# evroon/mav-detection

Hardware: NVIDIA B200
Metric: 1080p frame-pairs/sec (flow+FoE+mask) (higher is better)
Workload: dtype f32

## Files before the change

mav_detection_b200/csrc/api.cu:

```cuda
#include <math.h>
#include <stdarg.h>
#include <stdlib.h>
#include <string.h>

#include <algorithm>
#include <new>
#include <vector>

#include "common.cuh"

namespace mavd {

static thread_local char g_err[512] = "";
std::atomic<int64_t> g_launches{0};

void set_error(const char* fmt, ...) {
    va_list ap;
    va_start(ap, fmt);
    vsnprintf(g_err, sizeof(g_err), fmt, ap);
    va_end(ap);
}

static inline int cv_round(double v) { return (int)nearbyint(v); }

// ... 568 lines not shown
    pdl_break(h, 0);
    pdl_break(h, 1);
    MAVD_REQUIRE(n >= 0 && n <= h->cfg.max_pairs, MAVD_ERR_INVALID, "%s: batch %d exceeds max_pairs %d", what, n,
                 h->cfg.max_pairs);
    return MAVD_OK;
}

static void note_farneback_call(mavd_handle h, const uint8_t* d_frames, int n_pairs, int pair_stride, float* d_flow) {
    h->last_pairs = n_pairs;
    h->last_stride = pair_stride;
    h->last_flow0 = d_flow;
    h->last_frames = d_frames;
}

int mavd_farneback_tap(mavd_handle h, int32_t kind, int32_t level, int32_t index, float* d_out, void* stream) {
    MAVD_REQUIRE(h && d_out, MAVD_ERR_INVALID, "tap: NULL argument");
    DeviceGuard dg(h->cfg.device);
    MAVD_REQUIRE(index >= 0 && index < h->max_frames, MAVD_ERR_INVALID, "tap: index out of range");
    return farneback_tap(h, kind, level, index, d_out, (cudaStream_t)stream);
}

static int upload_imu(mavd_handle h, const mavd_imu* h_imu, int n, cudaStream_t s, int* n64, int* n32) {
    MAVD_REQUIRE(h_imu != nullptr, MAVD_ERR_INVALID, "imu array is NULL");
    int a = 0, b = 0, rot = 0;
    for (int i = 0; i < n; ++i) {
        if (h_imu[i].derotate) {
            MAVD_REQUIRE(h_imu[i].dt != 0.0, MAVD_ERR_INVALID, "imu[%d].dt is zero", i);
            ++a;
            if (!(h_imu[i].ang[0] == 0.0 && h_imu[i].ang[1] == 0.0 && h_imu[i].ang[2] == 0.0)) ++rot;
        } else {
            ++b;
        }
    }
    if (n64) *n64 = a;
    if (n32) *n32 = b;
    h->batch_rot = rot;
    const int k = h->imu_next;
    h->imu_next = (k + 1) % mavd_handle_s::kImuRing;
    MAVD_CUDA(cudaEventSynchronize(h->imu_ev[k]));
    mavd_imu* stage = h->h_imu_ring + (size_t)k * h->cfg.max_pairs;
    memcpy(stage, h_imu, sizeof(mavd_imu) * n);
    MAVD_CUDA(cudaMemcpyAsync(h->d_imu, stage, sizeof(mavd_imu) * n, cudaMemcpyHostToDevice, s));
    MAVD_CUDA(cudaEventRecord(h->imu_ev[k], s));
    return MAVD_OK;
}

int mavd_derotate(mavd_handle h, const float* d_flow, int32_t n, const mavd_imu* h_imu, double* d_out, void* stream) {
    DeviceGuard dg(h ? h->cfg.device : -1);
    TRY(check_batch(h, n, "derotate"));
    if (n == 0) return MAVD_OK;
    MAVD_REQUIRE(d_flow && d_out, MAVD_ERR_INVALID, "derotate: NULL buffer");
    TRY(upload_imu(h, h_imu, n, (cudaStream_t)stream, nullptr, nullptr));
    return derotate_run(h, d_flow, 0, n, h->d_imu, d_out, (cudaStream_t)stream);
}

int mavd_derotate_f64(mavd_handle h, const double* d_flow, int32_t n, const mavd_imu* h_imu, double* d_out, void* stream) {
    DeviceGuard dg(h ? h->cfg.device : -1);
    TRY(check_batch(h, n, "derotate_f64"));
    if (n == 0) return MAVD_OK;
// ... 51 lines not shown

int mavd_debug_force_exact_residual(mavd_handle h, int32_t on) {
    MAVD_REQUIRE(h != nullptr, MAVD_ERR_INVALID, "handle is NULL");
    DeviceGuard dg(h->cfg.device);
    MAVD_CUDA(cudaDeviceSynchronize());
    drop_graphs(h);
    h->force_exact_residual = on != 0;
    return MAVD_OK;
}

int mavd_residual_masks(mavd_handle h, const float* d_flow, int32_t n, const mavd_imu* h_imu,
                        const mavd_detect_params* prm, const double* d_foe, const uint8_t* d_sky, int64_t sky_stride,
                        const uint8_t* d_seg, int64_t seg_stride, void* d_phi, uint8_t* d_total, uint8_t* d_fixed,
                        mavd_frame_stats* d_stats, void* stream) {
    DeviceGuard dg(h ? h->cfg.device : -1);
    TRY(check_batch(h, n, "residual_masks"));
    if (n == 0) return MAVD_OK;
    MAVD_REQUIRE(d_flow && d_foe, MAVD_ERR_INVALID, "residual_masks: NULL buffer");
    mavd_detect_params p;
    if (prm) p = *prm; else mavd_default_detect_params(&p);
    int n64 = 0, n32 = 0;
    TRY(upload_imu(h, h_imu, n, (cudaStream_t)stream, &n64, &n32));
    return residual_run(h, d_flow, 0, n, h->d_imu, p, d_foe, d_sky, sky_stride, d_seg, seg_stride, d_phi, d_total, d_fixed,
                        d_stats, sizeof(mavd_frame_stats), n64 > 0 ? (h->batch_rot > 0 ? 1 : 2) : 0, n32 > 0, (cudaStream_t)stream);
}

static int check_det(mavd_handle h, int max_det, const void* det, const char* what) {
    if (!det) return MAVD_OK;
    MAVD_REQUIRE(max_det >= 1 && max_det <= MAVD_MAX_DETECTIONS, MAVD_ERR_INVALID, "%s: max_det %d outside 1..%d", what,
                 max_det, MAVD_MAX_DETECTIONS);
    MAVD_REQUIRE((reinterpret_cast<uintptr_t>(det) & 7) == 0, MAVD_ERR_INVALID, "%s: detections must be 8-byte aligned",
                 what);
    if (h->d_det_area) return MAVD_OK;
    mavd_handle_full* H = static_cast<mavd_handle_full*>(h);
    TRY(H->arena.alloc(&H->d_det_area, (size_t)h->cfg.max_pairs * det_lab_stride(h)));
    TRY(H->arena.alloc(&H->d_det_nlabels, (size_t)h->cfg.max_pairs));
    H->bytes = H->arena.bytes;
    return MAVD_OK;
}

int mavd_detections(mavd_handle h, const uint8_t* d_mask, int32_t n, const float* d_flow, const mavd_imu* h_imu,
                    int32_t max_det, mavd_detection* d_det, void* stream) {
    DeviceGuard dg(h ? h->cfg.device : -1);
    TRY(check_batch(h, n, "detections"));
    MAVD_REQUIRE(d_det != nullptr, MAVD_ERR_INVALID, "detections: NULL table");
    MAVD_REQUIRE(!d_flow || h_imu, MAVD_ERR_INVALID, "detections: a flow needs an imu array");
    TRY(check_det(h, max_det, d_det, "detections"));
// ... 69 lines not shown
static int detect_run(mavd_handle h, const float* flow, int n, const mavd_detect_params& p, int n64, int n32,
                      const int32_t* d_samples, const mavd_aux_inputs& aux, uint8_t* d_total_out, uint8_t* fixed,
                      mavd_frame_record* d_records, int max_det, mavd_detection* d_det, cudaStream_t s) {
    char* stats0 = reinterpret_cast<char*>(d_records) + offsetof(mavd_frame_record, stats);
    const bool fork = h->s_aux != nullptr && !h->prof.on;
    if (fork) {
        MAVD_CUDA(cudaEventRecord(h->ev_fork, s));
        MAVD_CUDA(cudaStreamWaitEvent(h->s_aux, h->ev_fork, 0));
        pdl_break(h, 1);
        TRY(ccl_list_reset(h, n, h->s_aux, 1));
        TRY(residual_prepare(h, n, aux.seg, aux.seg_stride, reinterpret_cast<mavd_frame_stats*>(stats0),
                             sizeof(mavd_frame_record), h->s_aux, 1));
        MAVD_CUDA(cudaEventRecord(h->ev_join, h->s_aux));
    }
    TRY(foe_run(h, flow, 0, n, h->d_imu, p, d_samples, h->d_foe, h->d_ninter, s));
    if (fork) {
        MAVD_CUDA(cudaStreamWaitEvent(s, h->ev_join, 0));
        pdl_break(h, 0);
    } else {
        TRY(ccl_list_reset(h, n, s));
    }
    TRY(residual_run(h, flow, 0, n, h->d_imu, p, h->d_foe, aux.sky, aux.sky_stride, aux.seg, aux.seg_stride, nullptr,
                     d_total_out, fixed, reinterpret_cast<mavd_frame_stats*>(stats0), sizeof(mavd_frame_record),
                     n64 > 0 ? (h->batch_rot > 0 ? 1 : 2) : 0, n32 > 0, s, true, aux.gt_flow, fork));
    int32_t* boxes0 = reinterpret_cast<int32_t*>(reinterpret_cast<char*>(d_records) + offsetof(mavd_frame_record, boxes));
    char* nl0 = reinterpret_cast<char*>(d_records) + offsetof(mavd_frame_record, n_labels);
    const DetArgs da{d_det, max_det, h->d_det_area, det_lab_stride(h), flow, h->d_imu};
    TRY(ccl_run(h, fixed, n, nullptr, boxes0, sizeof(mavd_frame_record) / sizeof(int32_t), MAVD_MAX_BOXES,
                reinterpret_cast<int32_t*>(nl0), sizeof(mavd_frame_record), s, true, d_det ? &da : nullptr));
    MAVD_CUDA(launch_chained(pdl_next(h), records_fill_kernel, ceil_div(n, 128), 128, 0, s, d_records, h->d_foe, h->d_ninter, n));
    MAVD_LAUNCHED();
    return MAVD_OK;
}

}

static constexpr size_t kMaxGraphs = 16;

struct KeyBuilder {
    std::vector<uint64_t> k;
    KeyBuilder& operator()(const void* p) { k.push_back((uint64_t)(uintptr_t)p); return *this; }
    KeyBuilder& operator()(int64_t v) { k.push_back((uint64_t)v); return *this; }
    KeyBuilder& operator()(const mavd_detect_params& p) {
        const size_t n = sizeof(p) / sizeof(uint64_t);
        uint64_t w[sizeof(mavd_detect_params) / sizeof(uint64_t)];
        memcpy(w, &p, sizeof(p));
        k.insert(k.end(), w, w + n);
// ... 95 lines not shown
    MAVD_REQUIRE(d_frames && d_flow, MAVD_ERR_INVALID, "farneback: NULL buffer");
    StreamScope ss(h, stream);
    note_farneback_call(h, d_frames, n_pairs, pair_stride, d_flow);
    return run_graphed(h, std::move(KeyBuilder()(int64_t(1))(d_frames)(int64_t(n_pairs))(int64_t(pair_stride))(d_flow).k),
                       ss.s, [&](cudaStream_t s) { return farneback_run(h, d_frames, n_pairs, pair_stride, d_flow, s); });
}

int mavd_detect_det(mavd_handle h, const float* d_flow, int32_t n, const mavd_imu* h_imu, const mavd_detect_params* prm,
                    const int32_t* d_samples, const mavd_aux_inputs* d_aux, uint8_t* d_total_out, uint8_t* d_fixed_out,
                    mavd_frame_record* d_records, int32_t max_det, mavd_detection* d_det, void* stream) {
    DeviceGuard dg(h ? h->cfg.device : -1);
    TRY(check_batch(h, n, "detect"));
    TRY(check_det(h, max_det, d_det, "detect"));
    if (!d_det) max_det = 0;
    if (n == 0) return MAVD_OK;
    MAVD_REQUIRE(d_flow && d_samples && d_records, MAVD_ERR_INVALID, "detect: NULL buffer");
    StreamScope ss(h, stream);
    mavd_detect_params p;
    if (prm) p = *prm; else mavd_default_detect_params(&p);
    const mavd_aux_inputs aux = d_aux ? *d_aux : kNoAux;
    int n64 = 0, n32 = 0;
    TRY(upload_imu(h, h_imu, n, ss.s, &n64, &n32));
    uint8_t* fixed = d_fixed_out ? d_fixed_out : h->d_fixed;
    return run_graphed(h, std::move(KeyBuilder()(int64_t(2))(d_flow)(int64_t(n))(p)(int64_t(n64))(int64_t(h->batch_rot > 0))(int64_t(n32))(d_samples)(aux)
                                        (d_total_out)(fixed)(d_records)(int64_t(max_det))(d_det).k),
                       ss.s, [&](cudaStream_t s) {
                           return detect_run(h, d_flow, n, p, n64, n32, d_samples, aux, d_total_out, fixed, d_records,
                                             max_det, d_det, s);
                       });
}

int mavd_detect_ex(mavd_handle h, const float* d_flow, int32_t n, const mavd_imu* h_imu, const mavd_detect_params* prm,
                   const int32_t* d_samples, const mavd_aux_inputs* d_aux, uint8_t* d_total_out, uint8_t* d_fixed_out,
                   mavd_frame_record* d_records, void* stream) {
    return mavd_detect_det(h, d_flow, n, h_imu, prm, d_samples, d_aux, d_total_out, d_fixed_out, d_records, 0, nullptr,
                           stream);
}

int mavd_detect(mavd_handle h, const float* d_flow, int32_t n, const mavd_imu* h_imu, const mavd_detect_params* prm,
                const int32_t* d_samples, const uint8_t* d_sky, int64_t sky_stride, const uint8_t* d_seg,
                int64_t seg_stride, uint8_t* d_total_out, uint8_t* d_fixed_out, mavd_frame_record* d_records,
                void* stream) {
    const mavd_aux_inputs aux = {d_sky, sky_stride, d_seg, seg_stride, nullptr};
    return mavd_detect_ex(h, d_flow, n, h_imu, prm, d_samples, &aux, d_total_out, d_fixed_out, d_records, stream);
}

int mavd_process_det(mavd_handle h, const uint8_t* d_frames, int32_t n_pairs, int32_t pair_stride, const mavd_imu* h_imu,
                     const mavd_detect_params* prm, const int32_t* d_samples, const mavd_aux_inputs* d_aux,
                     float* d_flow_out, uint8_t* d_total_out, uint8_t* d_fixed_out, mavd_frame_record* d_records,
                     int32_t max_det, mavd_detection* d_det, void* stream) {
    DeviceGuard dg(h ? h->cfg.device : -1);
    TRY(check_batch(h, n_pairs, "process"));
    MAVD_REQUIRE(pair_stride == 1 || pair_stride == 2, MAVD_ERR_INVALID, "pair_stride must be 1 or 2");
    TRY(check_det(h, max_det, d_det, "process"));
    if (!d_det) max_det = 0;
    if (n_pairs == 0) return MAVD_OK;
    MAVD_REQUIRE(d_frames && d_samples && d_records, MAVD_ERR_INVALID, "process: NULL buffer");
    StreamScope ss(h, stream);
    mavd_detect_params p;
    if (prm) p = *prm; else mavd_default_detect_params(&p);
    const mavd_aux_inputs aux = d_aux ? *d_aux : kNoAux;
    float* flow = d_flow_out ? d_flow_out : h->d_flow;
    uint8_t* fixed = d_fixed_out ? d_fixed_out : h->d_fixed;
    int n64 = 0, n32 = 0;
    TRY(upload_imu(h, h_imu, n_pairs, ss.s, &n64, &n32));
    note_farneback_call(h, d_frames, n_pairs, pair_stride, flow);
    return run_graphed(h, std::move(KeyBuilder()(int64_t(3))(d_frames)(int64_t(n_pairs))(int64_t(pair_stride))(p)(int64_t(n64))(int64_t(h->batch_rot > 0))
                                        (int64_t(n32))(d_samples)(aux)(flow)(d_total_out)(fixed)(d_records)(int64_t(max_det))
                                        (d_det).k),
                       ss.s, [&](cudaStream_t s) {
                           TRY(farneback_run(h, d_frames, n_pairs, pair_stride, flow, s));
                           return detect_run(h, flow, n_pairs, p, n64, n32, d_samples, aux, d_total_out, fixed, d_records,
                                             max_det, d_det, s);
                       });
}

int mavd_process_ex(mavd_handle h, const uint8_t* d_frames, int32_t n_pairs, int32_t pair_stride, const mavd_imu* h_imu,
                    const mavd_detect_params* prm, const int32_t* d_samples, const mavd_aux_inputs* d_aux,
                    float* d_flow_out, uint8_t* d_total_out, uint8_t* d_fixed_out, mavd_frame_record* d_records,
                    void* stream) {
    return mavd_process_det(h, d_frames, n_pairs, pair_stride, h_imu, prm, d_samples, d_aux, d_flow_out, d_total_out,
                            d_fixed_out, d_records, 0, nullptr, stream);
}

int mavd_process(mavd_handle h, const uint8_t* d_frames, int32_t n_pairs, int32_t pair_stride, const mavd_imu* h_imu,
                 const mavd_detect_params* prm, const int32_t* d_samples, const uint8_t* d_sky, int64_t sky_stride,
                 const uint8_t* d_seg, int64_t seg_stride, float* d_flow_out, uint8_t* d_total_out,
                 uint8_t* d_fixed_out, mavd_frame_record* d_records, void* stream) {
    const mavd_aux_inputs aux = {d_sky, sky_stride, d_seg, seg_stride, nullptr};
    return mavd_process_ex(h, d_frames, n_pairs, pair_stride, h_imu, prm, d_samples, &aux, d_flow_out, d_total_out,
// ... 278 lines not shown
```

mav_detection_b200/csrc/common.cuh:

```cuda
#pragma once
#include <cuda.h>
#include <cuda_runtime.h>
#include <stdint.h>
#include <stdio.h>
#include <atomic>
#include <vector>

#include "mavd.h"

namespace mavd {

void set_error(const char* fmt, ...);
extern std::atomic<int64_t> g_launches;

#define MAVD_CUDA(expr)                                                                         \
    do {                                                                                        \
        cudaError_t e__ = (expr);                                                               \
        if (e__ != cudaSuccess) {                                                               \
            ::mavd::set_error("%s:%d: %s -> %s", __FILE__, __LINE__, #expr, cudaGetErrorString(e__)); \
            return (e__ == cudaErrorMemoryAllocation) ? MAVD_ERR_NOMEM : MAVD_ERR_CUDA;          \
        }                                                                                       \
    } while (0)

#define MAVD_LAUNCHED()                                                                         \
// ... 181 lines not shown
        cudaEvent_t ev_in = nullptr, ev_done = nullptr, ev_out = nullptr;
        bool busy = false;
    } slot[MAVD_HOST_SLOTS];
    cudaStream_t s_in = nullptr, s_out = nullptr;
    cudaStream_t s_aux = nullptr;
    cudaEvent_t ev_fork = nullptr, ev_join = nullptr, ev_pyr = nullptr;
    mavd_tuning tune;
    mavd::Profiler prof;
    static constexpr int kImuRing = 8;
    mavd_imu* h_imu_ring = nullptr;
    cudaEvent_t imu_ev[kImuRing] = {};
    int imu_next = 0;
    struct GraphEntry {
        std::vector<uint64_t> key;
        cudaGraphExec_t exec = nullptr;
        int64_t launches = 0;
        uint64_t last_use = 0;
    };
    std::vector<GraphEntry> graphs;
    uint64_t graph_clock = 0;
    cudaStream_t s_main = nullptr;
    cudaEvent_t ev_main_in = nullptr, ev_main_out = nullptr;
    bool force_generic_iter = false;
    int batch_rot = 0;
    bool pdl_ok[2] = {false, false};
    int last_pairs = 0, last_stride = 1;
    float* last_flow0 = nullptr;
    const uint8_t* last_frames = nullptr;
};

namespace mavd {
static inline bool pdl_next(mavd_handle h, int lane = 0) {
    const bool chained = h->tune.use_pdl != 0 && !h->prof.on && h->pdl_ok[lane];
    h->pdl_ok[lane] = true;
    return chained;
}
static inline void pdl_break(mavd_handle h, int lane = 0) { h->pdl_ok[lane] = false; }

bool encode_tensor_map_3d(CUtensorMap* map, bool is_u8, const void* base, uint64_t d0, uint64_t d1, uint64_t d2,
                          uint64_t s1_bytes, uint64_t s2_bytes, uint32_t b0, uint32_t b1, uint32_t b2);
int farneback_run(mavd_handle h, const uint8_t* d_frames, int n_pairs, int pair_stride, float* d_flow,
                  cudaStream_t s);
int farneback_tap(mavd_handle h, int kind, int level, int index, float* d_out, cudaStream_t s);
int bgr2gray_run(const uint8_t* d_bgr, uint8_t* d_gray, int64_t n, cudaStream_t s);
int derotate_run(mavd_handle h, const void* d_flow, int flow_is_f64, int n, const mavd_imu* d_imu, double* d_out,
                 cudaStream_t s);
int foe_run(mavd_handle h, const void* d_flow, int flow_kind, int n, const mavd_imu* d_imu,
// ... 40 lines not shown
```

mav_detection_b200/csrc/detect.cu:

```cuda
#include <math.h>

#include <algorithm>

#include "common.cuh"

namespace mavd {

__global__ void __launch_bounds__(256) bgr2gray_kernel(const uint8_t* __restrict__ bgr, uint8_t* __restrict__ gray,
                                                      int64_t n) {
    int64_t i4 = ((int64_t)blockIdx.x * blockDim.x + threadIdx.x) * 4;
    if (i4 >= n) return;
    if (i4 + 4 <= n && ((uintptr_t)bgr & 3) == 0 && ((uintptr_t)gray & 3) == 0) {
        const uint32_t* p = reinterpret_cast<const uint32_t*>(bgr + i4 * 3);
        uint32_t a = __ldg(p), b = __ldg(p + 1), c = __ldg(p + 2);
        uint8_t v[12];
        v[0] = a; v[1] = a >> 8; v[2] = a >> 16; v[3] = a >> 24;
        v[4] = b; v[5] = b >> 8; v[6] = b >> 16; v[7] = b >> 24;
        v[8] = c; v[9] = c >> 8; v[10] = c >> 16; v[11] = c >> 24;
        uint32_t out = 0;
#pragma unroll
        for (int k = 0; k < 4; ++k) {
            uint32_t g = (v[3 * k] * 3735u + v[3 * k + 1] * 19235u + v[3 * k + 2] * 9798u + 16384u) >> 15;
            out |= g << (8 * k);
        }
        *reinterpret_cast<uint32_t*>(gray + i4) = out;
// ... 393 lines not shown
                                           bool& m_fixed) {
    const float a2 = fmaf(fx, fx, fy * fy), b2 = fmaf(dx, dx, dy * dy);
    const float ab2 = a2 * b2;
    const bool gt_dyn = a2 > p.dyn_mm2, gt_fix = a2 > p.fix_mm2;
    bool undecided = !(a2 < 1e15f) | !(b2 < 1e15f);
    undecided |= (fabsf(a2 - p.dyn_mm2) <= p.dyn_mm2_guard) | (fabsf(a2 - p.fix_mm2) <= p.fix_mm2_guard);
    const float dot = fmaf(fx, dx, fy * dy), crs = fabsf(fmaf(fx, dy, -(fy * dx)));
    const float sf = crs * p.fix_cos - dot * p.fix_sin;
    const float thr = fmaf(p.dyn_gain, rsqrtf(a2), p.dyn_c0);
    const float tr = thr * 0.017453292519943295f;
    float sn, cs;
    __sincosf(tr, &sn, &cs);
    const float sd = crs * cs - dot * sn;
    const float mf = 3.6e-5f, md = 3.6e-5f + 1e-5f * tr;
    undecided |= (gt_dyn | gt_fix) & (ab2 < 1e-8f);
    undecided |= gt_fix & (sf * sf <= (mf * mf) * ab2);
    undecided |= gt_dyn & ((sd * sd <= (md * md) * ab2) | !(thr < 170.f));
    m_fixed = gt_fix & (sf > 0.f);
    m_total = gt_dyn & (sd > 0.f);
    return !undecided;
}

constexpr int RES_ITEMS = 4;

template <int MODE, bool FAST, int VEC, int MINB = 4>
__global__ void __launch_bounds__(256, MINB) residual_kernel(const ResidualArgs A, const FastPrm fp) {
    pdl_entry();
    const int f = blockIdx.y;
    DerotRow dr;
    dr.on = 0;
    if (MODE != 2) {
        mavd_imu im;
        im.derotate = 0;
        if (A.imu) im = A.imu[f];
        if ((im.derotate != 0) != (MODE == 0)) return;
        if (MODE == 0) {
            __shared__ double s_dr[5];
            if (threadIdx.x < 3) s_dr[threadIdx.x] = __ddiv_rn(im.ang[threadIdx.x], im.dt);
            else if (threadIdx.x == 3) s_dr[3] = __ddiv_rn(__dmul_rn((double)A.w, im.dt), 2.0);
            else if (threadIdx.x == 4) s_dr[4] = __ddiv_rn(__dmul_rn((double)A.h, im.dt), 2.0);
            __syncthreads();
            dr.o0 = s_dr[0]; dr.o1 = s_dr[1]; dr.o2 = s_dr[2]; dr.s0 = s_dr[3]; dr.s1 = s_dr[4];
            dr.on = !(dr.o0 == 0.0 && dr.o1 == 0.0 && dr.o2 == 0.0 && fabs(dr.s0) < 1e300 && fabs(dr.s1) < 1e300);
        }
    }
    const int w = A.w, h = A.h;
    const int npx = w * h;
    const int ngrp = npx / VEC;
    const double foex = A.foe[2 * f], foey = A.foe[2 * f + 1];
    const size_t fbase = (size_t)f * npx;
    const uint8_t* sky = A.sky ? A.sky + (size_t)f * A.sky_stride : nullptr;
    const uint8_t* seg = A.seg ? A.seg + (size_t)f * A.seg_stride : nullptr;
    const bool want_stats = A.stats_base != nullptr;
    int seg_min = 0;
    if (seg && want_stats) {
        const double thr = 0.1 * (double)A.seg_max[f];
        seg_min = (int)floor(thr) + 1;
    }

    int c_tot = 0, c_fix = 0, c_pos = 0, c_tpt = 0, c_fpt = 0, c_tpf = 0, c_fpf = 0, n_px = 0;
    int bx0 = 0x7fffffff, by0 = 0x7fffffff, bx1 = -1, by1 = -1;
    double sfx = 0.0, sfy = 0.0, gfx = 0.0, gfy = 0.0, maxphi = 0.0;

#pragma unroll 1
    for (int it = 0; it < RES_ITEMS; ++it) {
        const int q = (blockIdx.x * RES_ITEMS + it) * 256 + threadIdx.x;
        if (q >= ngrp) break;
        const int i0 = q * VEC;
        const int y = A.row_magic ? (int)__umulhi((unsigned)i0, A.row_magic) : i0 / w, x0 = i0 - y * w;
        double vx[VEC], vy[VEC];
        float vfx[VEC], vfy[VEC];
        if (MODE == 2) {
            const double2* fl = reinterpret_cast<const double2*>(A.flow) + fbase + i0;
#pragma unroll
            for (int k = 0; k < VEC; ++k) { const double2 v = fl[k]; vx[k] = v.x; vy[k] = v.y; }
        } else if (VEC == 4) {
            const float4* fl = reinterpret_cast<const float4*>(reinterpret_cast<const float2*>(A.flow) + fbase + i0);
            const float4 u0 = __ldg(fl), u1 = __ldg(fl + 1);
            vfx[0] = u0.x; vfy[0] = u0.y; vfx[1] = u0.z; vfy[1] = u0.w;
            vfx[2] = u1.x; vfy[2] = u1.y; vfx[3] = u1.z; vfy[3] = u1.w;
        } else {
            const float2 v = reinterpret_cast<const float2*>(A.flow)[fbase + i0];
            vfx[0] = v.x; vfy[0] = v.y;
        }
        unsigned skyw = 0, segw = 0;
        if (VEC == 4) {
            if (sky) skyw = __ldg(reinterpret_cast<const unsigned*>(sky + i0));
            if (seg) segw = __ldg(reinterpret_cast<const unsigned*>(seg + i0));
        } else {
            if (sky) skyw = sky[i0];
            if (seg) segw = seg[i0];
        }
        double yn = 0.0;
        if (MODE == 0 && dr.on) yn = __ldg(A.yn + y);
        const float dyf = (float)((double)y - foey), dxf0 = (float)((double)x0 - foex);
        unsigned totw = 0, fixw = 0;
#pragma unroll
        for (int k = 0; k < VEC; ++k) {
            const int x = x0 + k;
            const bool not_sky = ((skyw >> (8 * k)) & 255u) == 0;
            bool mt = false, mf = false;
            if (MODE == 1) {
                float phi;
                pixel_exact_f32(vfx[k], vfy[k], x, y, foex, foey, A.prm, not_sky, mt, mf, phi);
                maxphi = fmax(maxphi, (double)phi);
                if (A.phi_out) reinterpret_cast<float*>(reinterpret_cast<double*>(A.phi_out) + fbase)[i0 + k] = phi;
            } else {
                double fdx = 0.0, fdy = 0.0;
                bool decided = false;
                if (FAST && MODE == 0 && !dr.on) {
                    decided = !not_sky;
                    if (!decided) decided = pixel_fast(vfx[k], vfy[k], dxf0 + (float)k, dyf, fp, mt, mf);
                    if (!decided) { fdx = (double)vfx[k]; fdy = (double)vfy[k]; }
                } else {
                    if (MODE == 0) {
                        fdx = vfx[k]; fdy = vfy[k];
                        if (dr.on) {
                            double r0, r1;
                            derot_tab(dr, __ldg(A.xn + x), yn, r0, r1);
                            fdx = __dsub_rn(fdx, r0);
                            fdy = __dsub_rn(fdy, r1);
                        }
                    } else {
                        fdx = vx[k]; fdy = vy[k];
                    }
                    vx[k] = fdx; vy[k] = fdy;
                    if (FAST) {
                        if (!not_sky) decided = true;
                        else decided = pixel_fast((float)fdx, (float)fdy, dxf0 + (float)k, dyf, fp, mt, mf);
                    }
                }
                if (!decided) {
                    double phi;
                    pixel_exact_f64(fdx, fdy, x, y, foex, foey, A.prm, not_sky, mt, mf, phi);
                    if (!FAST) {
                        maxphi = fmax(maxphi, phi);
                        if (A.phi_out) reinterpret_cast<double*>(A.phi_out)[fbase + i0 + k] = phi;
                    }
                }
            }
            totw |= (mt ? 1u : 0u) << (8 * k);
            fixw |= (mf ? 1u : 0u) << (8 * k);
        }
        if (A.unit_marks && fixw) {
            const int e = f * A.n_units + (i0 >> 7);
            if (*reinterpret_cast<volatile int*>(A.unit_marks + e) == 0 && atomicExch(A.unit_marks + e, 1) == 0)
                A.unit_list[atomicAdd(A.unit_count, 1)] = e;
        }
        n_px += VEC;
        if (want_stats && (totw | fixw | segw)) {
            c_tot += __popc(totw); c_fix += __popc(fixw);
            if (seg) {
                const unsigned live = VEC == 4 ? 0xffffffffu : 0xffu;
                const unsigned hi = segw & 0x80808080u & live;
                const unsigned nz = __vcmpne4(segw, 0u) & 0x01010101u & live;
                const unsigned n255 = __vcmpne4(segw, 0xffffffffu) & 0x01010101u & live;
                c_pos += __popc(hi);
                c_tpt += __popc(totw & nz); c_fpt += __popc(totw & n255);
                c_tpf += __popc(fixw & nz); c_fpf += __popc(fixw & n255);
                const unsigned smin = (unsigned)min(seg_min, 256);
                const unsigned ge = smin > 255u ? 0u : (__vcmpgeu4(segw, smin * 0x01010101u) & live);
                if (ge) {
                    bx0 = min(bx0, x0 + ((__ffs(ge) - 1) >> 3)); bx1 = max(bx1, x0 + ((31 - __clz(ge)) >> 3));
                    by0 = min(by0, y); by1 = max(by1, y);
                }
                if (hi) {
#pragma unroll
                    for (int k = 0; k < VEC; ++k)
                        if ((hi >> (8 * k)) & 0x80u) {
                            if (MODE == 1 || (FAST && MODE == 0 && !dr.on)) { sfx += (double)vfx[k]; sfy += (double)vfy[k]; }
                            else { sfx += vx[k]; sfy += vy[k]; }
                            if (MODE != 2 && A.gt_flow) {
                                const float2 g = __ldg(A.gt_flow + fbase + i0 + k);
                                double g0 = (double)g.x, g1 = (double)g.y;
                                if (MODE == 0 && dr.on) {
                                    double r0, r1;
                                    derot_tab(dr, __ldg(A.xn + x0 + k), yn, r0, r1);
                                    g0 = __dsub_rn(g0, r0);
                                    g1 = __dsub_rn(g1, r1);
                                }
                                gfx += g0; gfy += g1;
                            }
                        }
                }
            }
        }
        if (VEC == 4) {
            if (A.total_out) *reinterpret_cast<unsigned*>(A.total_out + fbase + i0) = totw;
            if (A.fixed_out) *reinterpret_cast<unsigned*>(A.fixed_out + fbase + i0) = fixw;
        } else {
            if (A.total_out) A.total_out[fbase + i0] = (uint8_t)totw;
            if (A.fixed_out) A.fixed_out[fbase + i0] = (uint8_t)fixw;
        }
    }
    if (!want_stats) return;

    __shared__ int s_cnt[8];
    __shared__ int s_bb[4];
    __shared__ double s_sum[4];
    __shared__ unsigned long long s_max;
    if (threadIdx.x < 8) s_cnt[threadIdx.x] = 0;
    if (threadIdx.x == 8) {
        s_bb[0] = s_bb[1] = 0x7fffffff; s_bb[2] = s_bb[3] = -1;
        s_sum[0] = s_sum[1] = s_sum[2] = s_sum[3] = 0.0; s_max = 0ull;
    }
    __syncthreads();
    const unsigned FULL = 0xffffffffu;
    const int lane = threadIdx.x & 31;
    c_tot = __reduce_add_sync(FULL, c_tot); c_fix = __reduce_add_sync(FULL, c_fix);
    if (lane == 0) { if (c_tot) atomicAdd(&s_cnt[0], c_tot); if (c_fix) atomicAdd(&s_cnt[1], c_fix); }
    if (!FAST) {
        unsigned long long mk = dmax_key(maxphi);
#pragma unroll
        for (int s = 16; s > 0; s >>= 1) {
            const unsigned long long t = __shfl_xor_sync(FULL, mk, s);
            mk = t > mk ? t : mk;
        }
// ... 60 lines not shown
__global__ void stats_init_kernel(char* stats_base, size_t stats_stride, int n, int* seg_max) {
    pdl_entry();
    int f = blockIdx.x * blockDim.x + threadIdx.x;
    if (f >= n) return;
    mavd_frame_stats* st = reinterpret_cast<mavd_frame_stats*>(stats_base + (size_t)f * stats_stride);
    mavd_frame_stats z;
    memset(&z, 0, sizeof(z));
    z.seg_bbox[0] = z.seg_bbox[1] = 0x7fffffff;
    z.seg_bbox[2] = z.seg_bbox[3] = -1;
    *st = z;
    if (seg_max) seg_max[f] = 0;
}

__global__ void stats_final_kernel(char* stats_base, size_t stats_stride, int n, int no_max_phi, const mavd_imu* imu) {
    pdl_entry();
    int f = blockIdx.x * blockDim.x + threadIdx.x;
    if (f >= n) return;
    mavd_frame_stats* st = reinterpret_cast<mavd_frame_stats*>(stats_base + (size_t)f * stats_stride);
    if (st->seg_bbox[2] < 0) st->seg_bbox[0] = st->seg_bbox[1] = st->seg_bbox[2] = st->seg_bbox[3] = -1;
    if (no_max_phi && (imu == nullptr || imu[f].derotate != 0)) st->max_phi = -1.0;
}

template <int MODE, bool FAST>
static int launch_residual(const ResidualArgs& A, const FastPrm& fp, int n, bool vec4, cudaStream_t s, bool pdl,
                           bool no_rotation = false) {
    const int npx = A.w * A.h;
    if (vec4 && no_rotation && MODE == 0 && FAST) {
        dim3 g(ceil_div(npx / 4, 256 * RES_ITEMS), n);
        MAVD_CUDA(launch_chained(pdl, residual_kernel<MODE, FAST, 4, (MODE == 0 && FAST) ? 5 : 4>, g, 256, 0, s, A, fp));
    } else if (vec4) {
        dim3 g(ceil_div(npx / 4, 256 * RES_ITEMS), n);
        MAVD_CUDA(launch_chained(pdl, residual_kernel<MODE, FAST, 4>, g, 256, 0, s, A, fp));
    } else {
        dim3 g(ceil_div(npx, 256 * RES_ITEMS), n);
        MAVD_CUDA(launch_chained(pdl, residual_kernel<MODE, FAST, 1>, g, 256, 0, s, A, fp));
    }
    MAVD_LAUNCHED();
    return MAVD_OK;
}

int residual_prepare(mavd_handle H, int n, const uint8_t* d_seg, int64_t seg_stride, mavd_frame_stats* d_stats,
                     size_t stats_stride, cudaStream_t s, int lane) {
    if (!d_stats) return MAVD_OK;
    ProfScope ps(&H->prof, MAVD_PROF_RESIDUAL, s);
    int* seg_max = reinterpret_cast<int*>(H->d_scan);
    MAVD_CUDA(launch_chained(pdl_next(H, lane), stats_init_kernel, ceil_div(n, 128), 128, 0, s, (char*)d_stats, stats_stride, n,
                             d_seg ? seg_max : nullptr));
    MAVD_LAUNCHED();
    if (d_seg) {
        dim3 g(32, n);
        MAVD_CUDA(launch_chained(pdl_next(H, lane), seg_max_kernel, g, 256, 0, s, d_seg, seg_stride,
                                 (int64_t)H->cfg.width * H->cfg.height, seg_max));
        MAVD_LAUNCHED();
// ... 23 lines not shown
    A.phi_out = d_phi; A.total_out = d_total; A.fixed_out = d_fixed;
    A.stats_base = (char*)d_stats; A.stats_stride = stats_stride;
    {
        const unsigned long long M = (1ull << 32) / (unsigned)w + 1, err = M * (unsigned)w - (1ull << 32);
        A.row_magic = (M < (1ull << 32) && (unsigned long long)npx * err < (1ull << 32)) ? (unsigned)M : 0u;
    }
    const bool listing = list_fixed_units && d_fixed != nullptr;
    A.unit_marks = listing ? ccl_unit_marks(H) : nullptr; A.unit_list = listing ? ccl_unit_list(H) : nullptr;
    A.unit_count = listing ? ccl_unit_count(H) : nullptr; A.n_units = ccl_n_units(H);
    auto gate_guard = [](double t) { const double g = 1e-5 * (t > 1.0 ? t : 1.0); return (float)(2.0 * t * g + g * g); };
    const double fixed_rad = p.fixed_angle * (3.14159265358979323846 / 180.0);
    const FastPrm fp{(float)(p.dyn_offset + p.dyn_base), (float)p.dyn_gain,
                     (float)(p.dyn_min_mag * p.dyn_min_mag), (float)(p.fixed_min_mag * p.fixed_min_mag),
                     gate_guard(p.dyn_min_mag), gate_guard(p.fixed_min_mag), (float)cos(fixed_rad), (float)sin(fixed_rad)};
    auto al = [](const void* q, uintptr_t a) { return q == nullptr || (reinterpret_cast<uintptr_t>(q) & (a - 1)) == 0; };
    const bool vec4 = (w % 4 == 0) && al(d_flow, 16) && al(d_sky, 4) && al(d_seg, 4) && al(d_total, 4) && al(d_fixed, 4) &&
                      (sky_stride % 4 == 0) && (seg_stride % 4 == 0);
    bool used_fast = false;
    if (flow_kind == 2) {
        if (fast) { used_fast = true; TRY_RC(launch_residual<2, true>(A, fp, n, vec4, s, pdl_next(H))); }
        else      TRY_RC(launch_residual<2, false>(A, fp, n, vec4, s, pdl_next(H)));
    } else {
        if (flow_kind == 0 && run_f64) {
            if (fast) { used_fast = true; TRY_RC(launch_residual<0, true>(A, fp, n, vec4, s, pdl_next(H), run_f64 == 2)); }
            else      TRY_RC(launch_residual<0, false>(A, fp, n, vec4, s, pdl_next(H)));
        }
        if (flow_kind == 1 || run_f32) TRY_RC(launch_residual<1, false>(A, fp, n, vec4, s, pdl_next(H)));
    }
    if (d_stats) {
        MAVD_CUDA(launch_chained(pdl_next(H), stats_final_kernel, ceil_div(n, 128), 128, 0, s, (char*)d_stats, stats_stride, n,
                                 used_fast ? 1 : 0, A.imu));
        MAVD_LAUNCHED();
    }
    return MAVD_OK;
}

__global__ void __launch_bounds__(256) magnitude_kernel(const void* __restrict__ flow, int is_f64, int64_t n,
                                                       void* __restrict__ out) {
    const int64_t i = (int64_t)blockIdx.x * blockDim.x + threadIdx.x;
    if (i >= n) return;
    if (is_f64) {
        const double2 v = reinterpret_cast<const double2*>(flow)[i];
        reinterpret_cast<double*>(out)[i] = __dsqrt_rn(__dadd_rn(__dmul_rn(v.x, v.x), __dmul_rn(v.y, v.y)));
    } else {
        const float2 v = reinterpret_cast<const float2*>(flow)[i];
        reinterpret_cast<float*>(out)[i] = __fsqrt_rn(__fadd_rn(__fmul_rn(v.x, v.x), __fmul_rn(v.y, v.y)));
    }
// ... 1192 lines not shown
```

Measured before the change: 5642.

## Defer undecided residual pixels to a post-pass and double-buffer loads in FAST kernel

The residual kernel is restructured so the FAST path records pixels the cheap f32 test cannot decide in a per-thread bitmask and resolves them afterwards with the exact f64 test, instead of doing that work inline. The derotation branch becomes a compile-time template via lambdas, and loads for the next group are double-buffered ahead of the current group's compute. The host-side zero-rotation counting, the batch_rot graph key and the special MINB=5 launch variant are removed. The intent is to keep rarely used f64 work out of the hot loop, which should lower register pressure and branch divergence and let loads overlap compute. The cost is extra scattered stores and a second flow read for each undecided pixel.

After: 5640 (median of 6 runs). Within noise of the previous version (-0.0%).

```diff
diff --git a/mav_detection_b200/csrc/api.cu b/mav_detection_b200/csrc/api.cu
--- a/mav_detection_b200/csrc/api.cu
+++ b/mav_detection_b200/csrc/api.cu
@@ -614,19 +614,17 @@
 
 static int upload_imu(mavd_handle h, const mavd_imu* h_imu, int n, cudaStream_t s, int* n64, int* n32) {
     MAVD_REQUIRE(h_imu != nullptr, MAVD_ERR_INVALID, "imu array is NULL");
-    int a = 0, b = 0, rot = 0;
+    int a = 0, b = 0;
     for (int i = 0; i < n; ++i) {
         if (h_imu[i].derotate) {
             MAVD_REQUIRE(h_imu[i].dt != 0.0, MAVD_ERR_INVALID, "imu[%d].dt is zero", i);
             ++a;
-            if (!(h_imu[i].ang[0] == 0.0 && h_imu[i].ang[1] == 0.0 && h_imu[i].ang[2] == 0.0)) ++rot;
         } else {
             ++b;
         }
     }
     if (n64) *n64 = a;
     if (n32) *n32 = b;
-    h->batch_rot = rot;
     const int k = h->imu_next;
     h->imu_next = (k + 1) % mavd_handle_s::kImuRing;
     MAVD_CUDA(cudaEventSynchronize(h->imu_ev[k]));
@@ -724,7 +722,7 @@
     int n64 = 0, n32 = 0;
     TRY(upload_imu(h, h_imu, n, (cudaStream_t)stream, &n64, &n32));
     return residual_run(h, d_flow, 0, n, h->d_imu, p, d_foe, d_sky, sky_stride, d_seg, seg_stride, d_phi, d_total, d_fixed,
-                        d_stats, sizeof(mavd_frame_stats), n64 > 0 ? (h->batch_rot > 0 ? 1 : 2) : 0, n32 > 0, (cudaStream_t)stream);
+                        d_stats, sizeof(mavd_frame_stats), n64 > 0, n32 > 0, (cudaStream_t)stream);
 }
 
 static int check_det(mavd_handle h, int max_det, const void* det, const char* what) {
@@ -840,7 +838,7 @@
     }
     TRY(residual_run(h, flow, 0, n, h->d_imu, p, h->d_foe, aux.sky, aux.sky_stride, aux.seg, aux.seg_stride, nullptr,
                      d_total_out, fixed, reinterpret_cast<mavd_frame_stats*>(stats0), sizeof(mavd_frame_record),
-                     n64 > 0 ? (h->batch_rot > 0 ? 1 : 2) : 0, n32 > 0, s, true, aux.gt_flow, fork));
+                     n64 > 0, n32 > 0, s, true, aux.gt_flow, fork));
     int32_t* boxes0 = reinterpret_cast<int32_t*>(reinterpret_cast<char*>(d_records) + offsetof(mavd_frame_record, boxes));
     char* nl0 = reinterpret_cast<char*>(d_records) + offsetof(mavd_frame_record, n_labels);
     const DetArgs da{d_det, max_det, h->d_det_area, det_lab_stride(h), flow, h->d_imu};
@@ -982,7 +980,7 @@
     int n64 = 0, n32 = 0;
     TRY(upload_imu(h, h_imu, n, ss.s, &n64, &n32));
     uint8_t* fixed = d_fixed_out ? d_fixed_out : h->d_fixed;
-    return run_graphed(h, std::move(KeyBuilder()(int64_t(2))(d_flow)(int64_t(n))(p)(int64_t(n64))(int64_t(h->batch_rot > 0))(int64_t(n32))(d_samples)(aux)
+    return run_graphed(h, std::move(KeyBuilder()(int64_t(2))(d_flow)(int64_t(n))(p)(int64_t(n64))(int64_t(n32))(d_samples)(aux)
                                         (d_total_out)(fixed)(d_records)(int64_t(max_det))(d_det).k),
                        ss.s, [&](cudaStream_t s) {
                            return detect_run(h, d_flow, n, p, n64, n32, d_samples, aux, d_total_out, fixed, d_records,
@@ -1025,7 +1023,7 @@
     int n64 = 0, n32 = 0;
     TRY(upload_imu(h, h_imu, n_pairs, ss.s, &n64, &n32));
     note_farneback_call(h, d_frames, n_pairs, pair_stride, flow);
-    return run_graphed(h, std::move(KeyBuilder()(int64_t(3))(d_frames)(int64_t(n_pairs))(int64_t(pair_stride))(p)(int64_t(n64))(int64_t(h->batch_rot > 0))
+    return run_graphed(h, std::move(KeyBuilder()(int64_t(3))(d_frames)(int64_t(n_pairs))(int64_t(pair_stride))(p)(int64_t(n64))
                                         (int64_t(n32))(d_samples)(aux)(flow)(d_total_out)(fixed)(d_records)(int64_t(max_det))
                                         (d_det).k),
                        ss.s, [&](cudaStream_t s) {
diff --git a/mav_detection_b200/csrc/common.cuh b/mav_detection_b200/csrc/common.cuh
--- a/mav_detection_b200/csrc/common.cuh
+++ b/mav_detection_b200/csrc/common.cuh
@@ -227,7 +227,6 @@
     cudaStream_t s_main = nullptr;
     cudaEvent_t ev_main_in = nullptr, ev_main_out = nullptr;
     bool force_generic_iter = false;
-    int batch_rot = 0;
     bool pdl_ok[2] = {false, false};
     int last_pairs = 0, last_stride = 1;
     float* last_flow0 = nullptr;
diff --git a/mav_detection_b200/csrc/detect.cu b/mav_detection_b200/csrc/detect.cu
--- a/mav_detection_b200/csrc/detect.cu
+++ b/mav_detection_b200/csrc/detect.cu
@@ -1,6 +1,7 @@
 #include <math.h>
 
 #include <algorithm>
+#include <type_traits>
 
 #include "common.cuh"
 
@@ -440,9 +441,43 @@
 }
 
 constexpr int RES_ITEMS = 4;
-
-template <int MODE, bool FAST, int VEC, int MINB = 4>
-__global__ void __launch_bounds__(256, MINB) residual_kernel(const ResidualArgs A, const FastPrm fp) {
+static_assert(RES_ITEMS * 4 <= 32, "the FAST path keeps one bit per pixel of a thread in a 32-bit word");
+
+template <int MODE, int VEC>
+struct ResIn {
+    float fx[MODE == 2 ? 1 : VEC], fy[MODE == 2 ? 1 : VEC];
+    double dx[MODE == 2 ? VEC : 1], dy[MODE == 2 ? VEC : 1];
+    unsigned skyw, segw;
+};
+
+template <int MODE, int VEC>
+__device__ __forceinline__ void res_load(ResIn<MODE, VEC>& g, const void* flow, const uint8_t* sky, const uint8_t* seg,
+                                         size_t fbase, int i0) {
+    if (MODE == 2) {
+        const double2* fl = reinterpret_cast<const double2*>(flow) + fbase + i0;
+#pragma unroll
+        for (int k = 0; k < VEC; ++k) { const double2 v = fl[k]; g.dx[k] = v.x; g.dy[k] = v.y; }
+    } else if (VEC == 4) {
+        const float4* fl = reinterpret_cast<const float4*>(reinterpret_cast<const float2*>(flow) + fbase + i0);
+        const float4 u0 = __ldg(fl), u1 = __ldg(fl + 1);
+        g.fx[0] = u0.x; g.fy[0] = u0.y; g.fx[1] = u0.z; g.fy[1] = u0.w;
+        g.fx[2] = u1.x; g.fy[2] = u1.y; g.fx[3] = u1.z; g.fy[3] = u1.w;
+    } else {
+        const float2 v = reinterpret_cast<const float2*>(flow)[fbase + i0];
+        g.fx[0] = v.x; g.fy[0] = v.y;
+    }
+    g.skyw = 0; g.segw = 0;
+    if (VEC == 4) {
+        if (sky) g.skyw = __ldg(reinterpret_cast<const unsigned*>(sky + i0));
+        if (seg) g.segw = __ldg(reinterpret_cast<const unsigned*>(seg + i0));
+    } else {
+        if (sky) g.skyw = sky[i0];
+        if (seg) g.segw = seg[i0];
+    }
+}
+
+template <int MODE, bool FAST, int VEC>
+__global__ void __launch_bounds__(256, 4) residual_kernel(const ResidualArgs A, const FastPrm fp) {
     pdl_entry();
     const int f = blockIdx.y;
     DerotRow dr;
@@ -476,96 +511,83 @@
         seg_min = (int)floor(thr) + 1;
     }
 
-    int c_tot = 0, c_fix = 0, c_pos = 0, c_tpt = 0, c_fpt = 0, c_tpf = 0, c_fpf = 0, n_px = 0;
+    int c_tot = 0, c_fix = 0, c_pos = 0, c_tpt = 0, c_fpt = 0, c_tpf = 0, c_fpf = 0;
+    unsigned und = 0;
     int bx0 = 0x7fffffff, by0 = 0x7fffffff, bx1 = -1, by1 = -1;
     double sfx = 0.0, sfy = 0.0, gfx = 0.0, gfy = 0.0, maxphi = 0.0;
-
-#pragma unroll 1
-    for (int it = 0; it < RES_ITEMS; ++it) {
-        const int q = (blockIdx.x * RES_ITEMS + it) * 256 + threadIdx.x;
-        if (q >= ngrp) break;
+    const unsigned smin4 = seg_min > 255 ? 0u : (unsigned)seg_min * 0x01010101u;
+
+    auto list_unit = [&](int i) {
+        const int e = f * A.n_units + (i >> 7);
+        if (*reinterpret_cast<volatile int*>(A.unit_marks + e) == 0 && atomicExch(A.unit_marks + e, 1) == 0)
+            A.unit_list[atomicAdd(A.unit_count, 1)] = e;
+    };
+
+    auto flow64 = [&](auto derot, const auto& g, int k, int x, double yn, double& fdx, double& fdy) {
+        if (MODE == 2) { fdx = g.dx[k]; fdy = g.dy[k]; return; }
+        fdx = (double)g.fx[k]; fdy = (double)g.fy[k];
+        if (decltype(derot)::value) {
+            double r0, r1;
+            derot_tab(dr, __ldg(A.xn + x), yn, r0, r1);
+            fdx = __dsub_rn(fdx, r0);
+            fdy = __dsub_rn(fdy, r1);
+        }
+    };
+
+    auto group = [&](auto derot, const ResIn<MODE, VEC>& g, int q, int ubit) {
+        constexpr bool DEROT = decltype(derot)::value;
         const int i0 = q * VEC;
         const int y = A.row_magic ? (int)__umulhi((unsigned)i0, A.row_magic) : i0 / w, x0 = i0 - y * w;
-        double vx[VEC], vy[VEC];
-        float vfx[VEC], vfy[VEC];
-        if (MODE == 2) {
-            const double2* fl = reinterpret_cast<const double2*>(A.flow) + fbase + i0;
-#pragma unroll
-            for (int k = 0; k < VEC; ++k) { const double2 v = fl[k]; vx[k] = v.x; vy[k] = v.y; }
-        } else if (VEC == 4) {
-            const float4* fl = reinterpret_cast<const float4*>(reinterpret_cast<const float2*>(A.flow) + fbase + i0);
-            const float4 u0 = __ldg(fl), u1 = __ldg(fl + 1);
-            vfx[0] = u0.x; vfy[0] = u0.y; vfx[1] = u0.z; vfy[1] = u0.w;
-            vfx[2] = u1.x; vfy[2] = u1.y; vfx[3] = u1.z; vfy[3] = u1.w;
-        } else {
-            const float2 v = reinterpret_cast<const float2*>(A.flow)[fbase + i0];
-            vfx[0] = v.x; vfy[0] = v.y;
-        }
-        unsigned skyw = 0, segw = 0;
-        if (VEC == 4) {
-            if (sky) skyw = __ldg(reinterpret_cast<const unsigned*>(sky + i0));
-            if (seg) segw = __ldg(reinterpret_cast<const unsigned*>(seg + i0));
-        } else {
-            if (sky) skyw = sky[i0];
-            if (seg) segw = seg[i0];
-        }
         double yn = 0.0;
-        if (MODE == 0 && dr.on) yn = __ldg(A.yn + y);
+        if (DEROT) yn = __ldg(A.yn + y);
         const float dyf = (float)((double)y - foey), dxf0 = (float)((double)x0 - foex);
         unsigned totw = 0, fixw = 0;
-#pragma unroll
-        for (int k = 0; k < VEC; ++k) {
-            const int x = x0 + k;
-            const bool not_sky = ((skyw >> (8 * k)) & 255u) == 0;
-            bool mt = false, mf = false;
-            if (MODE == 1) {
-                float phi;
-                pixel_exact_f32(vfx[k], vfy[k], x, y, foex, foey, A.prm, not_sky, mt, mf, phi);
-                maxphi = fmax(maxphi, (double)phi);
-                if (A.phi_out) reinterpret_cast<float*>(reinterpret_cast<double*>(A.phi_out) + fbase)[i0 + k] = phi;
-            } else {
-                double fdx = 0.0, fdy = 0.0;
-                bool decided = false;
-                if (FAST && MODE == 0 && !dr.on) {
-                    decided = !not_sky;
-                    if (!decided) decided = pixel_fast(vfx[k], vfy[k], dxf0 + (float)k, dyf, fp, mt, mf);
-                    if (!decided) { fdx = (double)vfx[k]; fdy = (double)vfy[k]; }
+        if (FAST && MODE == 0 && !DEROT) {
+            const unsigned lit = VEC == 4 ? __vcmpeq4(g.skyw, 0u) : (g.skyw == 0 ? 1u : 0u);
+            if (lit) {
+#pragma unroll
+                for (int k = 0; k < VEC; ++k) {
+                    bool mt, mf;
+                    const bool decided = pixel_fast(g.fx[k], g.fy[k], dxf0 + (float)k, dyf, fp, mt, mf);
+                    const bool not_sky = (lit >> (8 * k)) & 1u;
+                    und |= (not_sky && !decided ? 1u : 0u) << (ubit + k);
+                    totw |= (not_sky && decided && mt ? 1u : 0u) << (8 * k);
+                    fixw |= (not_sky && decided && mf ? 1u : 0u) << (8 * k);
+                }
+            }
+        } else {
+#pragma unroll
+            for (int k = 0; k < VEC; ++k) {
+                const int x = x0 + k;
+                const bool not_sky = ((g.skyw >> (8 * k)) & 255u) == 0;
+                bool mt = false, mf = false;
+                if (MODE == 1) {
+                    float phi;
+                    pixel_exact_f32(g.fx[k], g.fy[k], x, y, foex, foey, A.prm, not_sky, mt, mf, phi);
+                    maxphi = fmax(maxphi, (double)phi);
+                    if (A.phi_out) reinterpret_cast<float*>(reinterpret_cast<double*>(A.phi_out) + fbase)[i0 + k] = phi;
+                } else if (FAST) {
+                    if (not_sky) {
+                        double fdx, fdy;
+                        flow64(derot, g, k, x, yn, fdx, fdy);
+                        if (!pixel_fast((float)fdx, (float)fdy, dxf0 + (float)k, dyf, fp, mt, mf)) {
+                            und |= 1u << (ubit + k);
+                            mt = mf = false;
+                        }
+                    }
                 } else {
-                    if (MODE == 0) {
-                        fdx = vfx[k]; fdy = vfy[k];
-                        if (dr.on) {
-                            double r0, r1;
-                            derot_tab(dr, __ldg(A.xn + x), yn, r0, r1);
-                            fdx = __dsub_rn(fdx, r0);
-                            fdy = __dsub_rn(fdy, r1);
-                        }
-                    } else {
-                        fdx = vx[k]; fdy = vy[k];
-                    }
-                    vx[k] = fdx; vy[k] = fdy;
-                    if (FAST) {
-                        if (!not_sky) decided = true;
-                        else decided = pixel_fast((float)fdx, (float)fdy, dxf0 + (float)k, dyf, fp, mt, mf);
-                    }
+                    double fdx, fdy, phi;
+                    flow64(derot, g, k, x, yn, fdx, fdy);
+                    pixel_exact_f64(fdx, fdy, x, y, foex, foey, A.prm, not_sky, mt, mf, phi);
+                    maxphi = fmax(maxphi, phi);
+                    if (A.phi_out) reinterpret_cast<double*>(A.phi_out)[fbase + i0 + k] = phi;
                 }
-                if (!decided) {
-                    double phi;
-                    pixel_exact_f64(fdx, fdy, x, y, foex, foey, A.prm, not_sky, mt, mf, phi);
-                    if (!FAST) {
-                        maxphi = fmax(maxphi, phi);
-                        if (A.phi_out) reinterpret_cast<double*>(A.phi_out)[fbase + i0 + k] = phi;
-                    }
-                }
-            }
-            totw |= (mt ? 1u : 0u) << (8 * k);
-            fixw |= (mf ? 1u : 0u) << (8 * k);
-        }
-        if (A.unit_marks && fixw) {
-            const int e = f * A.n_units + (i0 >> 7);
-            if (*reinterpret_cast<volatile int*>(A.unit_marks + e) == 0 && atomicExch(A.unit_marks + e, 1) == 0)
-                A.unit_list[atomicAdd(A.unit_count, 1)] = e;
-        }
-        n_px += VEC;
+                totw |= (mt ? 1u : 0u) << (8 * k);
+                fixw |= (mf ? 1u : 0u) << (8 * k);
+            }
+        }
+        if (A.unit_marks && fixw) list_unit(i0);
+        const unsigned segw = g.segw;
         if (want_stats && (totw | fixw | segw)) {
             c_tot += __popc(totw); c_fix += __popc(fixw);
             if (seg) {
@@ -576,8 +598,7 @@
                 c_pos += __popc(hi);
                 c_tpt += __popc(totw & nz); c_fpt += __popc(totw & n255);
                 c_tpf += __popc(fixw & nz); c_fpf += __popc(fixw & n255);
-                const unsigned smin = (unsigned)min(seg_min, 256);
-                const unsigned ge = smin > 255u ? 0u : (__vcmpgeu4(segw, smin * 0x01010101u) & live);
+                const unsigned ge = smin4 ? (__vcmpgeu4(segw, smin4) & live) : 0u;
                 if (ge) {
                     bx0 = min(bx0, x0 + ((__ffs(ge) - 1) >> 3)); bx1 = max(bx1, x0 + ((31 - __clz(ge)) >> 3));
                     by0 = min(by0, y); by1 = max(by1, y);
@@ -586,12 +607,13 @@
 #pragma unroll
                     for (int k = 0; k < VEC; ++k)
                         if ((hi >> (8 * k)) & 0x80u) {
-                            if (MODE == 1 || (FAST && MODE == 0 && !dr.on)) { sfx += (double)vfx[k]; sfy += (double)vfy[k]; }
-                            else { sfx += vx[k]; sfy += vy[k]; }
+                            double fdx, fdy;
+                            flow64(derot, g, k, x0 + k, yn, fdx, fdy);
+                            sfx += fdx; sfy += fdy;
                             if (MODE != 2 && A.gt_flow) {
-                                const float2 g = __ldg(A.gt_flow + fbase + i0 + k);
-                                double g0 = (double)g.x, g1 = (double)g.y;
-                                if (MODE == 0 && dr.on) {
+                                const float2 gt = __ldg(A.gt_flow + fbase + i0 + k);
+                                double g0 = (double)gt.x, g1 = (double)gt.y;
+                                if (DEROT) {
                                     double r0, r1;
                                     derot_tab(dr, __ldg(A.xn + x0 + k), yn, r0, r1);
                                     g0 = __dsub_rn(g0, r0);
@@ -610,7 +632,62 @@
             if (A.total_out) A.total_out[fbase + i0] = (uint8_t)totw;
             if (A.fixed_out) A.fixed_out[fbase + i0] = (uint8_t)fixw;
         }
-    }
+    };
+
+    const int q0 = blockIdx.x * (RES_ITEMS * 256) + threadIdx.x;
+    auto run = [&](auto derot) {
+        constexpr bool DEROT = decltype(derot)::value;
+        ResIn<MODE, VEC> ga, gb;
+        if (!FAST) {
+#pragma unroll 1
+            for (int it = 0; it < RES_ITEMS; ++it) {
+                const int q = q0 + it * 256;
+                if (q >= ngrp) break;
+                res_load(ga, A.flow, sky, seg, fbase, q * VEC);
+                group(derot, ga, q, it * VEC);
+            }
+            return;
+        }
+        if (q0 < ngrp) res_load(ga, A.flow, sky, seg, fbase, q0 * VEC);
+#pragma unroll 1
+        for (int it = 0; it < RES_ITEMS; it += 2) {
+            const int q = q0 + it * 256;
+            if (q >= ngrp) break;
+            const bool more = q + 256 < ngrp;
+            if (more) res_load(gb, A.flow, sky, seg, fbase, (q + 256) * VEC);
+            group(derot, ga, q, it * VEC);
+            if (!more) break;
+            if (it + 2 < RES_ITEMS && q + 512 < ngrp) res_load(ga, A.flow, sky, seg, fbase, (q + 512) * VEC);
+            group(derot, gb, q + 256, (it + 1) * VEC);
+        }
+        while (und) {
+            const int b = __ffs(und) - 1;
+            und &= und - 1;
+            const int i = (q0 + (b / VEC) * 256) * VEC + b % VEC;
+            const int y = A.row_magic ? (int)__umulhi((unsigned)i, A.row_magic) : i / w, x = i - y * w;
+            ResIn<MODE, 1> g1;
+            res_load(g1, A.flow, nullptr, nullptr, fbase, i);
+            double fdx, fdy, phi;
+            flow64(derot, g1, 0, x, DEROT ? __ldg(A.yn + y) : 0.0, fdx, fdy);
+            bool mt, mf;
+            pixel_exact_f64(fdx, fdy, x, y, foex, foey, A.prm, true, mt, mf, phi);
+            if (!(mt || mf)) continue;
+            if (mt && A.total_out) A.total_out[fbase + i] = 1;
+            if (mf && A.fixed_out) A.fixed_out[fbase + i] = 1;
+            if (mf && A.unit_marks) list_unit(i);
+            if (want_stats) {
+                c_tot += mt; c_fix += mf;
+                if (seg) {
+                    const unsigned gv = seg[i];
+                    c_tpt += mt && gv != 0; c_fpt += mt && gv != 255;
+                    c_tpf += mf && gv != 0; c_fpf += mf && gv != 255;
+                }
+            }
+        }
+    };
+    if (MODE == 0 && dr.on) run(std::true_type{});
+    else run(std::false_type{});
+    const int n_px = q0 < ngrp ? min(RES_ITEMS, (ngrp - q0 + 255) / 256) * VEC : 0;
     if (!want_stats) return;
 
     __shared__ int s_cnt[8];
@@ -717,13 +794,9 @@
 }
 
 template <int MODE, bool FAST>
-static int launch_residual(const ResidualArgs& A, const FastPrm& fp, int n, bool vec4, cudaStream_t s, bool pdl,
-                           bool no_rotation = false) {
+static int launch_residual(const ResidualArgs& A, const FastPrm& fp, int n, bool vec4, cudaStream_t s, bool pdl) {
     const int npx = A.w * A.h;
-    if (vec4 && no_rotation && MODE == 0 && FAST) {
-        dim3 g(ceil_div(npx / 4, 256 * RES_ITEMS), n);
-        MAVD_CUDA(launch_chained(pdl, residual_kernel<MODE, FAST, 4, (MODE == 0 && FAST) ? 5 : 4>, g, 256, 0, s, A, fp));
-    } else if (vec4) {
+    if (vec4) {
         dim3 g(ceil_div(npx / 4, 256 * RES_ITEMS), n);
         MAVD_CUDA(launch_chained(pdl, residual_kernel<MODE, FAST, 4>, g, 256, 0, s, A, fp));
     } else {
@@ -793,7 +866,7 @@
         else      TRY_RC(launch_residual<2, false>(A, fp, n, vec4, s, pdl_next(H)));
     } else {
         if (flow_kind == 0 && run_f64) {
-            if (fast) { used_fast = true; TRY_RC(launch_residual<0, true>(A, fp, n, vec4, s, pdl_next(H), run_f64 == 2)); }
+            if (fast) { used_fast = true; TRY_RC(launch_residual<0, true>(A, fp, n, vec4, s, pdl_next(H))); }
             else      TRY_RC(launch_residual<0, false>(A, fp, n, vec4, s, pdl_next(H)));
         }
         if (flow_kind == 1 || run_f32) TRY_RC(launch_residual<1, false>(A, fp, n, vec4, s, pdl_next(H)));
```
